# autosome-ru/pasio

Measured on NVIDIA B200. Metric: whole-contig segmentation throughput, default pasio pipeline (nt/s); DP cell updates/s in dp_cells_per_s, higher is better.
Workload: dtype f64

## Files before the change

pasio_b200/csrc/window_dp.cu:

```cuda
#include "dp_core.cuh"
#include "bound.cuh"
#include <cstdio>
#include <cstdlib>

namespace {

constexpr int WD_THREADS = 256;
constexpr int WD_WARPS = WD_THREADS / 32;
constexpr int WD_FARW = WD_WARPS - 1;
constexpr int NEAR_Q = 4;
constexpr int PR_CB = 32;
constexpr int PR_FB = 8;
constexpr int PR_MIN_N = 256;
constexpr int PR_DENSE = 28;

#ifdef PASIO_WD_PROF
__device__ unsigned long long g_wd_prof[16];
struct ProfAcc { long long t0; long long a0, a1, a2, a3, a4, a5, a6, a7; };
#define PROF_DECL ProfAcc prof = {clock64(), 0, 0, 0, 0, 0, 0, 0, 0}
__device__ __forceinline__ long long prof_clock()
{
    unsigned dummy;
    long long t;
    asm volatile("ld.volatile.shared.u32 %0, [%1];" : "=r"(dummy) : "r"(0u) : "memory");
    asm volatile("mov.u64 %0, %%clock64;" : "=l"(t) : "r"(dummy) : "memory");
    return t;
}
#define PROF_T(i) do { const long long t1__ = prof_clock(); prof.a##i += t1__ - prof.t0; prof.t0 = t1__; } while (0)
#define PROF_FLUSH do { if (threadIdx.x == 0 || threadIdx.x == 32) { unsigned long long *g__ = g_wd_prof + (threadIdx.x ? 8 : 0); \
    atomicAdd(g__ + 0, (unsigned long long)prof.a0); atomicAdd(g__ + 1, (unsigned long long)prof.a1); \
    atomicAdd(g__ + 2, (unsigned long long)prof.a2); atomicAdd(g__ + 3, (unsigned long long)prof.a3); \
    atomicAdd(g__ + 4, (unsigned long long)prof.a4); atomicAdd(g__ + 5, (unsigned long long)prof.a5); \
    atomicAdd(g__ + 6, (unsigned long long)prof.a6); atomicAdd(g__ + 7, (unsigned long long)prof.a7); } \
    prof.a0 = prof.a1 = prof.a2 = prof.a3 = prof.a4 = prof.a5 = prof.a6 = prof.a7 = 0; } while (0)
#define PROF_ARGS , ProfAcc &prof
#define PROF_PASS , prof
#else
#define PROF_DECL
#define PROF_T(i) do { } while (0)
#define PROF_FLUSH do { } while (0)
#define PROF_ARGS
#define PROF_PASS
#endif

struct WinDpParams {
    WinGeom geom;
    i64 nwin;
    const int32_t *cand;
    const i64 *cg;
    const i64 *cgc;
    const uint32_t *cpbits;
    uint32_t *keepbits;
    const double *gtab;
    const double *ltab;
    int constraint;
    int alpha_int;
    double alpha;
    double pen;
    int cap;
    u64 *cells;
    u64 *cells_skipped;
    unsigned *work_counter;
    const int32_t *list;
    i64 w_begin;
    i64 n_p1, list_len;
    unsigned char *done_flags;
    int p1_stride;
    int skip_covered;
    int speculate;
    int n_lg;
};

__host__ __device__ inline size_t window_smem_bytes(int cap)
{
    const size_t capr = (size_t)((cap + 31) & ~31);
    return capr * 16
           + NEAR_Q * 32 * 8
           + DP_JB * DP_JB * 8
           + NEAR_Q * 32 * 4
           + 24 * 4
           + capr * 2
           + (capr / PR_CB) * sizeof(CoarseRec)
           + 2 * 32 * sizeof(float4)
           + capr * 2
           + 2 * ((capr / PR_CB) * 2 + 16)
           + 2 * WD_FARW * 32 * (8 + 4)
           + 8 * 8;
}

__device__ __forceinline__ int2 col_lc(const ColRec *sCol, int i)
{
    return *reinterpret_cast<const int2 *>(sCol + i);
}

template <bool AI>
__device__ __forceinline__ void compute_row_lb(int jbp, int jb, int N, const ColRec *sCol, float4 *sRow, double *sRowStat,
                                               double delta_path, double pen,
                                               const double *__restrict__ gtab, const double *__restrict__ ltab,
                                               int alpha_int, double alpha)
{
    const int lane = threadIdx.x & 31;
    const int jrow = min(jb + lane, N - 1);
    const int2 me = col_lc(sCol, jrow);
    const RowConst<AI> rme = make_row<AI>(me.y, me.x, alpha_int, alpha);
    const int jp = jbp + lane;
    const int2 pm = col_lc(sCol, jp), pb = col_lc(sCol, jp - 1), before = col_lc(sCol, jrow - 1);
    const RowConst<AI> rp = make_row<AI>(pm.y, pm.x, alpha_int, alpha);
    const double wp = self_score<AI>(pb.y, pb.x, rp, gtab, ltab) + pen;
    double run = self_score<AI>(before.y, before.x, rme, gtab, ltab) + (lane ? pen : 0.0);
    const double tot_prev = warp_sum(wp);
#pragma unroll
    for (int d = 1; d < 32; d <<= 1) {
        const double o = __shfl_up_sync(0xffffffffu, run, d);
        if (lane >= d) run += o;
    }
    double path = (sCol[jbp - 1].P + tot_prev) + run - delta_path;
    if (!(fabs(path) < 1e30)) path = -INFINITY;
    float lbf = (float)path;
    sRow[lane] = make_float4(lbf, (float)me.y, (float)me.x, 0.f);
    double ab = (jb + lane < N && path > -1e300) ? fabs(path) : 0.0;
#pragma unroll
    for (int off = 16; off > 0; off >>= 1) ab = fmax(ab, __shfl_xor_sync(0xffffffffu, ab, off));
    if (lane == 0) *sRowStat = ab;
}

__device__ __forceinline__ double tilted_row_min(const float4 *sRow, int r0, int r1, double a, double b, double lbabs,
                                                 int c_max, int l_max)
{
    const float af = (float)a, bf = (float)b;
    float m = INFINITY;
#pragma unroll 4
    for (int r = r0; r <= r1; ++r) {
        const float4 rr = sRow[r];
        m = fminf(m, fmaf(af, rr.y, fmaf(bf, rr.z, rr.x)));
    }
    const double err = (lbabs + fabs(a) * (double)c_max + fabs(b) * (double)l_max) * 9.5367431640625e-07;
    return (double)m - err;
}

template <bool AI>
__device__ __forceinline__ u64 far_pass(int jb, int N, int nfar, const ColRec *sCol, const CoarseRec *sCoarse,
                                        const float4 *sRow, double lbabs, unsigned short *sList, unsigned short *sDense,
                                        unsigned short *sSurv, int *sListCount ,
                                        double *sFarVW, int *sFarAW, double delta,
                                        const double *__restrict__ gtab, const double *__restrict__ ltab,
                                        int alpha_int, double alpha PROF_ARGS)
{
    const int lane = threadIdx.x & 31, w7 = (threadIdx.x >> 5) - 1;
    const int nrows = min(DP_JB, N - jb);
    const int2 rowF = col_lc(sCol, jb), rowL = col_lc(sCol, jb + nrows - 1);
    const int2 me = col_lc(sCol, min(jb + lane, N - 1));
    const RowConst<AI> rme = make_row<AI>(me.y, me.x, alpha_int, alpha);

    double best = -INFINITY;
    int arg = 0x7fffffff;
    if (w7 == 0 && lane < nrows) {
        const ColRec a0 = sCol[0];
        best = __dadd_rn(self_score<AI>(a0.C, a0.L, rme, gtab, ltab), a0.P);
        arg = 0;
    }
    u64 skipped = 0;

    const int rg = lane >> 2, q = lane & 3;
    const int r0 = 4 * rg, r1 = min(r0 + 3, nrows - 1);
    const bool act2 = r0 < nrows;
    const int2 gF = col_lc(sCol, jb + min(r0, nrows - 1)), gL = col_lc(sCol, jb + r1);

    auto level2 = [&](int cb1) {
        const CoarseRec *rec = sCoarse + cb1;
        const double a = rec->a, b = rec->b;
        bool surv2 = false;
        if (act2) {
            const int i0 = 1 + PR_CB * cb1 + PR_FB * q;
            const int2 cF = col_lc(sCol, i0), cL = col_lc(sCol, i0 + PR_FB - 1);
            const double m2 = tilted_box_max<AI>(gF.y - cL.y, gL.y - cF.y, gF.x - cL.x, gL.x - cF.x, a, b,
                                                 gtab, ltab, alpha_int, alpha);
            const double m3 = tilted_row_min(sRow, r0, r1, a, b, lbabs, gL.y, gL.x);
            surv2 = !(rec->mpt8[q] + m2 - m3 + delta < 0.0);
            if (!surv2) skipped += (u64)(PR_FB * (r1 - r0 + 1));
        }
        const unsigned mask2 = __ballot_sync(0xffffffffu, surv2);
        const int n2 = __popc(mask2);
        if (n2 >= PR_DENSE) {
            if (act2 && !surv2) skipped -= (u64)(PR_FB * (r1 - r0 + 1));
            if (lane == 0) sDense[atomicAdd(sListCount + 1, 1)] = (unsigned short)cb1;
        } else if (n2) {
            int slot = 0;
            if (lane == 0) slot = atomicAdd(sListCount, n2);
            slot = __shfl_sync(0xffffffffu, slot, 0);
            if (surv2) sList[slot + __popc(mask2 & ((1u << lane) - 1u))] = (unsigned short)((cb1 << 5) | lane);
        }
    };
    const int l1_warps = min(WD_FARW, (nfar + 31) / 32);
    const int n_direct = max(0, min(nfar, WD_FARW - l1_warps));
    const int nfar1 = nfar - n_direct;
    if (w7 >= l1_warps && w7 - l1_warps < n_direct) level2(nfar - 1 - (w7 - l1_warps));

    for (int base = 0; base + 32 * w7 < nfar1 && w7 < l1_warps; base += 32 * l1_warps) {
        const int cb = base + 32 * w7 + lane;
        bool surv1 = false;
        if (cb < nfar1) {
            const CoarseRec *rec = sCoarse + cb;
            const int4 ends = *reinterpret_cast<const int4 *>(rec);
            const double a1 = rec->a, b1 = rec->b;
            const double ub1 = rec->mpt + tilted_box_max<AI>(rowF.y - ends.y, rowL.y - ends.x, rowF.x - ends.w, rowL.x - ends.z,
                                                             a1, b1, gtab, ltab, alpha_int, alpha);
            const double m3 = tilted_row_min(sRow, 0, nrows - 1, a1, b1, lbabs, rowL.y, rowL.x);
            surv1 = !(ub1 - m3 + delta < 0.0);
            if (!surv1) skipped += (u64)(PR_CB * nrows);
        }
        const unsigned mask1 = __ballot_sync(0xffffffffu, surv1);
        if (mask1) {
            int slot = 0;
            if (lane == 0) slot = atomicAdd(sListCount + 2, __popc(mask1));
            slot = __shfl_sync(0xffffffffu, slot, 0);
            if (surv1) sSurv[slot + __popc(mask1 & ((1u << lane) - 1u))] = (unsigned short)cb;
        }
    }
    PROF_T(4);
    asm volatile("bar.sync 1, %0;" ::"n"(WD_FARW * 32) : "memory");
    const int nsurv = *reinterpret_cast<volatile int *>(sListCount + 2);

    for (int e = w7; e < nsurv; e += WD_FARW) level2(sSurv[e]);
    PROF_T(5);
    asm volatile("bar.sync 1, %0;" ::"n"(WD_FARW * 32) : "memory");
    const int total = *reinterpret_cast<volatile int *>(sListCount);
    const int ndense = *reinterpret_cast<volatile int *>(sListCount + 1);
    PROF_T(3);

    for (int e = w7; e < ndense; e += WD_FARW) {
        const int i0 = 1 + PR_CB * (int)sDense[e];
        const int rr = lane & 3, cph = lane >> 2;
#pragma unroll 1
        for (int g = 0; g < 4; ++g) {
            RowConst<AI> r[2];
            double bst[2];
            int ag[2];
#pragma unroll
            for (int k = 0; k < 2; ++k) {
                const int2 rl = col_lc(sCol, min(jb + g * 8 + k * 4 + rr, N - 1));
                r[k] = make_row<AI>(rl.y, rl.x, alpha_int, alpha);
                bst[k] = -INFINITY;
                ag[k] = i0 + cph;
            }
            sweep_columns<AI, 4, 2>(i0, i0 + PR_CB, cph, 8, sCol, r, gtab, ltab, bst, ag);
#pragma unroll
            for (int k = 0; k < 2; ++k) {
                merge_column_phases<4>(bst[k], ag[k]);
                const double v = __shfl_sync(0xffffffffu, bst[k], lane & 3);
                const int va = __shfl_sync(0xffffffffu, ag[k], lane & 3);
                if ((lane >> 2) == g * 2 + k && lane < nrows && (v > best || (v == best && va < arg))) { best = v; arg = va; }
            }
        }
    }

    constexpr int UX = 4;
    const int er = lane >> 3, ec = lane & 7;
    for (int e0 = w7 * UX; e0 < total; e0 += WD_FARW * UX) {
        double t[UX];
        int ta[UX], g4[UX];
#pragma unroll
        for (int u = 0; u < UX; ++u) {
            t[u] = -INFINITY;
            ta[u] = 0x7fffffff;
            g4[u] = 0;
            if (e0 + u < total) {
                const int ent = sList[e0 + u];
                const int l2 = ent & 31;
                g4[u] = 4 * (l2 >> 2);
                const int row = g4[u] + er;
                const int col = 1 + PR_CB * (ent >> 5) + PR_FB * (l2 & 3) + ec;
                ta[u] = col;
                if (row < nrows) {
                    const int2 rl = col_lc(sCol, jb + row);
                    const RowConst<AI> rc = make_row<AI>(rl.y, rl.x, alpha_int, alpha);
                    const ColRec cc = sCol[col];
                    t[u] = __dadd_rn(self_score<AI>(cc.C, cc.L, rc, gtab, ltab), cc.P);
                }
            }
        }
#pragma unroll
        for (int u = 0; u < UX; ++u) {
#pragma unroll
            for (int off = 1; off < 8; off <<= 1) {
                const double ob = __shfl_xor_sync(0xffffffffu, t[u], off);
                const int oa = __shfl_xor_sync(0xffffffffu, ta[u], off);
                if (ob > t[u] || (ob == t[u] && oa < ta[u])) { t[u] = ob; ta[u] = oa; }
            }
            const int rel = lane - g4[u];
            const double v = __shfl_sync(0xffffffffu, t[u], (rel & 3) * 8);
            const int va = __shfl_sync(0xffffffffu, ta[u], (rel & 3) * 8);
            if (rel >= 0 && rel < 4 && (v > best || (v == best && va < arg))) { best = v; arg = va; }
        }
    }
    sFarVW[lane] = best;
    sFarAW[lane] = arg;
    return skipped;
}

template <bool AI, int NW>
__device__ __forceinline__ void near_tri_farwarps(int w7 , int jb, int N, const ColRec *sCol, double *sPartV,
                                                  int *sPartA, double *sTri,
                                                  const double *__restrict__ gtab, const double *__restrict__ ltab,
                                                  int alpha_int, double alpha)
{
    const int lane = threadIdx.x & 31;
    const int rr = lane & 3, cc = lane >> 2;
    constexpr int NT = (16 + NW - 1) / NW;
    double tv[NT][2];
    int tcol[NT];
#pragma unroll
    for (int u = 0; u < NT; ++u) {
        const int t = w7 + u * NW;
        const int grp = t & 3, qc = (t >> 2) & 3;
        tcol[u] = jb - PR_CB + qc * 8 + cc;
        const ColRec a = sCol[tcol[u]];
#pragma unroll
        for (int k = 0; k < 2; ++k) {
            const int j = min(jb + grp * 8 + k * 4 + rr, N - 1);
            const int2 me = col_lc(sCol, j);
            const RowConst<AI> r = make_row<AI>(me.y, me.x, alpha_int, alpha);
            tv[u][k] = (t < 16) ? __dadd_rn(self_score<AI>(a.C, a.L, r, gtab, ltab), a.P) : -INFINITY;
        }
    }
    const int2 mt = col_lc(sCol, min(jb + lane, N - 1));
    const RowConst<AI> rt = make_row<AI>(mt.y, mt.x, alpha_int, alpha);
    constexpr int NK = (DP_JB + NW - 1) / NW;
    double w[NK];
#pragma unroll
    for (int kk = 0; kk < NK; ++kk) {
        const int k = w7 + kk * NW;
        w[kk] = 0.0;
        if (k < lane && jb + lane < N) {
            const int2 a = col_lc(sCol, jb + k);
            w[kk] = self_score<AI>(a.y, a.x, rt, gtab, ltab);
        }
    }
#pragma unroll
    for (int u = 0; u < NT; ++u) {
        const int t = w7 + u * NW;
#pragma unroll
        for (int k = 0; k < 2; ++k) {
            double best = tv[u][k];
            int arg = tcol[u];
            merge_column_phases<4>(best, arg);
            if (cc == 0 && t < 16) {
                const int row = (t & 3) * 8 + k * 4 + rr;
                sPartV[(t >> 2) * 32 + row] = best;
                sPartA[(t >> 2) * 32 + row] = arg;
            }
        }
    }
#pragma unroll
    for (int kk = 0; kk < NK; ++kk) {
        const int k = w7 + kk * NW;
        if (k < lane && jb + lane < N) sTri[k * DP_JB + lane] = w[kk];
    }
}

__device__ __forceinline__ void build_coarse_record(int jb, const ColRec *sCol, CoarseRec *rec, double tilt_scale_c,
                                                    double tilt_scale_l)
{
    const ColRec me = sCol[jb + (threadIdx.x & 31)];
    fit_column_record(me.C, me.L, me.P, rec, tilt_scale_c, tilt_scale_l);
}

template <bool AI, int U, int RPL, bool PRUNE>
__global__ void __launch_bounds__(WD_THREADS, 3)
window_dp_kernel(WinDpParams p)
{
    extern __shared__ __align__(16) unsigned char smem[];
    const int capr = (p.cap + 31) & ~31;
    ColRec *sCol = reinterpret_cast<ColRec *>(smem);
    double *sPartV = reinterpret_cast<double *>(sCol + capr);
    double *sTri = sPartV + NEAR_Q * 32;
    int *sPartA = reinterpret_cast<int *>(sTri + DP_JB * DP_JB);
    int *sMisc = sPartA + NEAR_Q * 32;
    unsigned short *sPrev = reinterpret_cast<unsigned short *>(sMisc + 24);
    CoarseRec *sCoarse = reinterpret_cast<CoarseRec *>(sPrev + capr);
    float4 *sRow = reinterpret_cast<float4 *>(sCoarse + capr / PR_CB);
    double *sFarV = reinterpret_cast<double *>(sRow + 2 * 32);
    int *sFarA = reinterpret_cast<int *>(sFarV + 2 * WD_FARW * 32);
    double *sScal = reinterpret_cast<double *>(sFarA + 2 * WD_FARW * 32);
    unsigned short *sList = reinterpret_cast<unsigned short *>(sScal + 8);
    int *sListCount = sMisc + 16;
    unsigned short *sJump = reinterpret_cast<unsigned short *>(sCoarse);
    unsigned char *sMark = reinterpret_cast<unsigned char *>(sTri);

    const int tid = threadIdx.x, lane = tid & 31, warp = tid >> 5;
    PROF_DECL;

    while (true) {
        PROF_T(7);
        PROF_FLUSH;
        if (tid == 0) sMisc[0] = (int)atomicAdd(p.work_counter, 1u);
        __syncthreads();
        const i64 widx = (unsigned)sMisc[0];
        if (widx >= p.nwin) break;
        const bool second = widx >= p.n_p1;
        const bool phase2 = second && p.skip_covered;
        const i64 w = !p.list ? p.w_begin + widx
                              : (second ? (i64)__ldg(p.list + (p.list_len - 1 - (widx - p.n_p1))) : (i64)__ldg(p.list + widx));
        if (phase2) {
            if (tid == 0) {
                const i64 rel = w - p.w_begin, lo = rel - rel % p.p1_stride, hi = lo + p.p1_stride;
                const volatile unsigned char *f = p.done_flags;
                while (!f[lo] || (hi < p.list_len && !f[hi])) __nanosleep(200);
                __threadfence();
                i64 skip_cells = -1;
                if (hi < p.list_len && (f[lo] & 2) && (f[hi] & 2)) {
                    i64 s0, e0, s1, e1, s2, e2;
                    window_range(p.geom, w, s0, e0);
                    window_range(p.geom, p.w_begin + lo, s1, e1);
                    window_range(p.geom, p.w_begin + hi, s2, e2);
                    if (s1 <= s0 && e1 >= s2 && e2 >= e0) skip_cells = (e0 - s0) * (e0 - s0 - 1) / 2;
                }
                if (skip_cells >= 0) {
                    atomicAdd(p.cells, (u64)skip_cells);
                    atomicAdd(p.cells_skipped, (u64)skip_cells);
                }
                sMisc[1] = skip_cells >= 0;
            }
            __syncthreads();
            if (sMisc[1]) continue;
        }
        int kept_all = 1;

        i64 st, en;
        window_range(p.geom, w, st, en);
        const int nq = (int)(en - st);
        const i64 first = p.cand ? (i64)__ldg(p.cand + st) : st;
        const i64 last = p.cand ? (i64)__ldg(p.cand + en - 1) : en - 1;
        const i64 cg_first = p.cand ? __ldg(p.cgc + st) : __ldg(p.cg + first);
        const bool all_zero = (p.constraint == PASIO_CONSTRAINT_ZEROS) && ((p.cand ? __ldg(p.cgc + en - 1) : __ldg(p.cg + last)) == cg_first);
        int count = 0;
        const bool by_words = !p.cand && p.constraint == PASIO_CONSTRAINT_CONSTANTS;
        if (by_words) {
            const i64 w0 = first >> 5, w1 = last >> 5;
            const int nwords = (int)(w1 - w0 + 1);
            for (int base = 0; base < nwords; base += WD_THREADS) {
                const int t = base + tid;
                unsigned word = 0;
                if (t < nwords) {
                    word = __ldg(p.cpbits + w0 + t);
                    if (t == 0) word = (word & (0xffffffffu << (first & 31))) | (1u << (first & 31));
                    if (t == nwords - 1) word = (word & (0xffffffffu >> (31 - (last & 31)))) | (1u << (last & 31));
                }
                int incl = __popc(word);
                const int mine = incl;
#pragma unroll
                for (int d = 1; d < 32; d <<= 1) {
                    const int o = __shfl_up_sync(0xffffffffu, incl, d);
                    if (lane >= d) incl += o;
                }
                if (lane == 31) sMisc[4 + warp] = incl;
                __syncthreads();
                int woff = 0, tot = 0;
#pragma unroll
                for (int w2 = 0; w2 < WD_WARPS; ++w2) {
                    const int c = sMisc[4 + w2];
                    if (w2 < warp) woff += c;
                    tot += c;
                }
                int k = count + woff + incl - mine;
                const i64 pos0 = (w0 + t) << 5;
                while (word) {
                    const i64 pos = pos0 + (__ffs(word) - 1);
                    word &= word - 1;
                    sCol[k].L = (int)(pos - first);
                    sCol[k].C = (int)(__ldg(p.cg + pos) - cg_first);
                    ++k;
                }
                count += tot;
                __syncthreads();
            }
        }
        for (int base = 0; !by_words && base < nq; base += WD_THREADS) {
            const int q = base + tid;
            i64 pos = 0;
            bool take = false;
            if (q < nq) {
                pos = p.cand ? (i64)__ldg(p.cand + st + q) : st + q;
                if (q == 0 || q == nq - 1 || p.constraint == PASIO_CONSTRAINT_NONE) take = true;
                else if (p.constraint == PASIO_CONSTRAINT_CONSTANTS) take = bit_test(p.cpbits, pos);
                else take = !all_zero;
                if (phase2 && !((__ldcg(p.keepbits + (pos >> 5)) >> (pos & 31)) & 1u)) kept_all = 0;
            }
            const unsigned bal = __ballot_sync(0xffffffffu, take);
            if (lane == 0) sMisc[4 + warp] = __popc(bal);
            __syncthreads();
            int woff = 0, tot = 0;
#pragma unroll
            for (int w2 = 0; w2 < WD_WARPS; ++w2) {
                const int c = sMisc[4 + w2];
                if (w2 < warp) woff += c;
                tot += c;
            }
            if (take) {
                const int k = count + woff + __popc(bal & ((1u << lane) - 1u));
                sCol[k].L = (int)(pos - first);
                sCol[k].C = (int)((p.cand ? __ldg(p.cgc + st + q) : __ldg(p.cg + pos)) - cg_first);
            }
            count += tot;
            __syncthreads();
        }
        const int N = count;
        PROF_T(0);
        if (phase2 && __syncthreads_and(kept_all)) {
            if (tid == 0) {
                const u64 c = (u64)N * (u64)(N - 1) / 2;
                atomicAdd(p.cells, c);
                atomicAdd(p.cells_skipped, c);
            }
            continue;
        }

        if (tid == 0) { sCol[0].P = 0.0; sPrev[0] = 0; }
        __syncthreads();
        u64 skipped = 0;
        if (PRUNE && tid == 0) {
            const ColRec z = sCol[N - 1];
            const int x = z.C + (AI ? p.alpha_int : 0);
            sScal[0] = fabs(__ldg(p.gtab + x)) + ((double)z.C + p.alpha) * fabs(__ldg(p.ltab + z.L)) + 1.0;
            sScal[1] = 0.0;
            sScal[2] = (double)z.C + p.alpha;
            sScal[3] = (double)z.L;
        }
        auto finish_block = [&](int jb) {
            if (jb + DP_JB <= N) build_coarse_record(jb, sCol, sCoarse + (jb - 1) / PR_CB, sScal[2], sScal[3]);
            double ab = jb + lane < N ? fabs(sCol[jb + lane].P) : 0.0;
#pragma unroll
            for (int off = 16; off > 0; off >>= 1) ab = fmax(ab, __shfl_xor_sync(0xffffffffu, ab, off));
            if (lane == 0) sScal[1] = fmax(sScal[1], ab);
        };
        auto far_delta = [&]() { return (sScal[0] + sScal[1] + fabs(p.pen) * DP_JB) * 5.684341886080802e-14; };
        auto prepare_rows = [&](int jbn) {
            const int par = ((jbn - 1) / DP_JB) & 1;
            const double delta_path = (sScal[0] + sScal[1] + fabs(p.pen) * DP_JB) * 1.8189894035458565e-12;
            compute_row_lb<AI>(jbn - DP_JB, jbn, N, sCol, sRow + 32 * par, sScal + 4 + par, delta_path, p.pen, p.gtab, p.ltab,
                               p.alpha_int, p.alpha);
            if (lane == 0) { sListCount[4 * par] = 0; sListCount[4 * par + 1] = 0; sListCount[4 * par + 2] = 0; }
        };
        auto run_far = [&](int jbf) {
            const int kf = (jbf - 1) / DP_JB, par = kf & 1;
            skipped += far_pass<AI>(jbf, N, kf - 1, sCol, sCoarse, sRow + 32 * par, sScal[4 + par], sList, sList + capr,
                                    sList + capr + capr / PR_CB + 8, sListCount + 4 * par, sFarV + (par * WD_FARW + warp - 1) * 32,
                                    sFarA + (par * WD_FARW + warp - 1) * 32,
                                    far_delta(), p.gtab, p.ltab, p.alpha_int, p.alpha PROF_PASS);
        };
        int jb = 1;
        const bool pipelined = PRUNE && N > PR_MIN_N && p.cand != nullptr;
        for (; jb < N && (!pipelined || jb < 1 + 2 * DP_JB); jb += DP_JB) {
            dp_block_step<AI, WD_WARPS, U, RPL>(jb, N, 0, sCol, sPrev, nullptr, sPartV, sPartA, sTri,
                                                p.gtab, p.ltab, p.alpha_int, p.alpha, p.pen, -INFINITY, 0, 0);
            if (pipelined && warp == 0) finish_block(jb);
        }
        PROF_T(6);
        if (pipelined && jb < N) {
            int spec_wait = 0, spec_back = 1;
            if (warp == 0) prepare_rows(jb);
            __syncthreads();
            if (warp > 0) run_far(jb);
            else if (jb + DP_JB < N) prepare_rows(jb + DP_JB);
            __syncthreads();
            for (; jb < N; jb += DP_JB) {
                const int k = (jb - 1) / DP_JB, buf = k & 1;
                near_tri_farwarps<AI, WD_WARPS>(warp, jb, N, sCol, sPartV, sPartA, sTri, p.gtab, p.ltab, p.alpha_int, p.alpha);
                PROF_T(1);
                __syncthreads();
                PROF_T(6);
                if (warp == 0) {
                    double fbest = -INFINITY;
                    int farg = 0;
#pragma unroll
                    for (int w2 = 0; w2 < WD_FARW; ++w2) {
                        const double v = sFarV[(buf * WD_FARW + w2) * 32 + lane];
                        const int a = sFarA[(buf * WD_FARW + w2) * 32 + lane];
                        if (v > fbest || (v == fbest && a < farg)) { fbest = v; farg = a; }
                    }
                    const double ib = jb + lane < N ? fbest : -INFINITY;
                    const int ia = jb + lane < N ? farg : 0;
                    bool resolved = false;
                    if (p.speculate && spec_wait == 0) {
                        resolved = block_chain_speculative<NEAR_Q>(jb, N, sCol, sPrev, sPartV, sPartA, sTri, p.pen, ib, ia);
                        if (resolved) spec_back = 1;
                        else { spec_wait = spec_back; spec_back = min(spec_back * 2, 16); }
                    } else if (spec_wait > 0) {
                        --spec_wait;
                    }
                    if (!resolved) block_chain<NEAR_Q>(jb, N, sCol, sPrev, nullptr, sPartV, sPartA, sTri, p.pen, ib, ia, 0, nullptr);
                    __syncwarp();
                    finish_block(jb);
                    if (jb + 2 * DP_JB < N) prepare_rows(jb + 2 * DP_JB);
                } else if (jb + DP_JB < N) {
                    run_far(jb + DP_JB);
                }
                PROF_T(2);
                __syncthreads();
                PROF_T(7);
            }
        }

        for (int k = tid; k < N; k += WD_THREADS) sMark[k] = (k == N - 1);
        __syncthreads();
        unsigned short *ja = sPrev, *jb2 = sJump;
        for (int reach = 1; reach < N; reach <<= 1) {
            for (int k = tid; k < N; k += WD_THREADS)
                if (sMark[k]) sMark[ja[k]] = 1;
            for (int k = tid; k < N; k += WD_THREADS) jb2[k] = ja[ja[k]];
            __syncthreads();
            unsigned short *t = ja; ja = jb2; jb2 = t;
        }
        int every = N == nq;
        for (int k = tid; k < N; k += WD_THREADS) {
            if (sMark[k]) {
                const i64 pos = first + sCol[k].L;
                atomicOr(p.keepbits + (pos >> 5), 1u << (pos & 31));
            } else {
                every = 0;
            }
        }
        if (!second && p.skip_covered && p.n_p1 < p.nwin) {
            __threadfence();
            every = __syncthreads_and(every);
            if (tid == 0) {
                __threadfence();
                *reinterpret_cast<volatile unsigned char *>(p.done_flags + (w - p.w_begin)) = every ? 3 : 1;
            }
        }
        if (tid == 0) atomicAdd(p.cells, (u64)N * (u64)(N - 1) / 2);
        if (PRUNE) {
#pragma unroll
            for (int off = 16; off > 0; off >>= 1) skipped += __shfl_xor_sync(0xffffffffu, skipped, off);
            if (lane == 0 && skipped) atomicAdd(p.cells_skipped, skipped);
        }
        __syncthreads();
    }
}

constexpr int SW_JB = 16;
constexpr int SW_SMALL_N = WD_SMALL_MAX_CANDIDATES, SW_SMALL_WARPS = 8, SW_SMALL_CTAS = 5;
constexpr int SW_MEDIUM_N = WD_MEDIUM_MAX_CANDIDATES, SW_MEDIUM_WARPS = 4, SW_MEDIUM_CTAS = 4;

template <int MAXN>
struct __align__(16) SmallWin {
    ColRec col[MAXN];
    double tri[SW_JB * SW_JB];
    unsigned short prev[MAXN];
    unsigned char mark[MAXN];
};

template <bool AI, int MAXN, int NWARPS, int CTAS, int U, bool LGS>
__global__ void __launch_bounds__(NWARPS * 32, CTAS)
small_window_dp_kernel(WinDpParams p)
{
    extern __shared__ __align__(16) unsigned char smem[];
    const int lane = threadIdx.x & 31;
    SmallWin<MAXN> &W = reinterpret_cast<SmallWin<MAXN> *>(smem)[threadIdx.x >> 5];
    u64 my_cells = 0;
    const double *lgt = p.ltab;
    if (LGS) {
        double *sLg = reinterpret_cast<double *>(smem + sizeof(SmallWin<MAXN>) * NWARPS);
        for (int k = threadIdx.x; k < p.n_lg; k += NWARPS * 32) sLg[k] = __ldg(p.ltab + k);
        __syncthreads();
        lgt = sLg;
    }

    while (true) {
        unsigned widx = 0;
        if (lane == 0) widx = atomicAdd(p.work_counter, 1u);
        widx = __shfl_sync(0xffffffffu, widx, 0);
        if ((i64)widx >= p.nwin) break;
        const i64 w = __ldg(p.list + widx);

        i64 st, en;
        window_range(p.geom, w, st, en);
        const int nq = (int)(en - st);
        const i64 first = p.cand ? (i64)__ldg(p.cand + st) : st;
        const i64 last = p.cand ? (i64)__ldg(p.cand + en - 1) : en - 1;
        const i64 cg_first = p.cand ? __ldg(p.cgc + st) : __ldg(p.cg + first);
        const bool all_zero = (p.constraint == PASIO_CONSTRAINT_ZEROS) && ((p.cand ? __ldg(p.cgc + en - 1) : __ldg(p.cg + last)) == cg_first);
        int count = 0;
        if (!p.cand && p.constraint == PASIO_CONSTRAINT_CONSTANTS) {
            const i64 w0 = first >> 5, w1 = last >> 5;
            const int nwords = (int)(w1 - w0 + 1);
            for (int base = 0; base < nwords; base += 32) {
                const int t = base + lane;
                unsigned word = 0;
                if (t < nwords) {
                    word = __ldg(p.cpbits + w0 + t);
                    if (t == 0) word = (word & (0xffffffffu << (first & 31))) | (1u << (first & 31));
                    if (t == nwords - 1) word = (word & (0xffffffffu >> (31 - (last & 31)))) | (1u << (last & 31));
                }
                int incl = __popc(word);
                const int mine = incl;
#pragma unroll
                for (int d = 1; d < 32; d <<= 1) {
                    const int o = __shfl_up_sync(0xffffffffu, incl, d);
                    if (lane >= d) incl += o;
                }
                int k = count + incl - mine;
                const i64 pos0 = (w0 + t) << 5;
                while (word) {
                    const i64 pos = pos0 + (__ffs(word) - 1);
                    word &= word - 1;
                    W.col[k].L = (int)(pos - first);
                    W.col[k].C = (int)(__ldg(p.cg + pos) - cg_first);
                    ++k;
                }
                count += __shfl_sync(0xffffffffu, incl, 31);
            }
        } else {
            for (int base = 0; base < nq; base += 32) {
                const int q = base + lane;
                i64 pos = 0;
                bool take = false;
                if (q < nq) {
                    pos = p.cand ? (i64)__ldg(p.cand + st + q) : st + q;
                    if (q == 0 || q == nq - 1 || p.constraint == PASIO_CONSTRAINT_NONE) take = true;
                    else if (p.constraint == PASIO_CONSTRAINT_CONSTANTS) take = bit_test(p.cpbits, pos);
                    else take = !all_zero;
                }
                const unsigned bal = __ballot_sync(0xffffffffu, take);
                if (take) {
                    const int k = count + __popc(bal & ((1u << lane) - 1u));
                    W.col[k].L = (int)(pos - first);
                    W.col[k].C = (int)((p.cand ? __ldg(p.cgc + st + q) : __ldg(p.cg + pos)) - cg_first);
                }
                count += __popc(bal);
            }
        }
        const int N = count;
        if (lane == 0) { W.col[0].P = 0.0; W.prev[0] = 0; }
        __syncwarp();

        const int r = lane & 15, ph = lane >> 4;
        for (int jb = 1; jb < N; jb += SW_JB) {
            const ColRec me = W.col[min(jb + r, N - 1)];
            RowConst<AI> rc[1] = {make_row<AI>(me.C, me.L, p.alpha_int, p.alpha)};
            double best[1] = {-INFINITY};
            int arg[1] = {ph};
            sweep_columns<AI, U, 1, LGS>(0, jb, ph, 2, W.col, rc, p.gtab, lgt, best, arg);
            {
                const double ob = __shfl_xor_sync(0xffffffffu, best[0], 16);
                const int oa = __shfl_xor_sync(0xffffffffu, arg[0], 16);
                if (ob > best[0] || (ob == best[0] && oa < arg[0])) { best[0] = ob; arg[0] = oa; }
            }
            for (int k = ph; k < r; k += 2)
                if (jb + r < N) {
                    const ColRec a = W.col[jb + k];
                    W.tri[k * SW_JB + r] = self_score<AI, LGS>(a.C, a.L, rc[0], p.gtab, lgt);
                }
            __syncwarp();
            double bst = best[0], mine = 0.0;
            int ag = arg[0];
            const int rows = min(SW_JB, N - jb);
#pragma unroll 4
            for (int k = 0; k < rows; ++k) {
                const double pf = __dadd_rn(bst, p.pen);
                const double pk = __shfl_sync(0xffffffffu, pf, k);
                if (r == k) mine = pf;
                if (r > k) {
                    const double t = __dadd_rn(W.tri[k * SW_JB + r], pk);
                    if (t > bst) { bst = t; ag = jb + k; }
                }
            }
            if (lane < SW_JB && jb + r < N) {
                W.col[jb + r].P = mine;
                W.prev[jb + r] = (unsigned short)ag;
            }
            __syncwarp();
        }

        for (int k = lane; k < N; k += 32) W.mark[k] = 0;
        __syncwarp();
        if (lane == 0) {
            int k = N - 1;
            while (true) {
                W.mark[k] = 1;
                if (k == 0) break;
                k = W.prev[k];
            }
        }
        __syncwarp();
        for (int k = lane; k < N; k += 32)
            if (W.mark[k]) {
                const i64 pos = first + W.col[k].L;
                atomicOr(p.keepbits + (pos >> 5), 1u << (pos & 31));
            }
        my_cells += (u64)N * (u64)(N - 1) / 2;
        __syncwarp();
    }
    if (lane == 0 && my_cells) atomicAdd(p.cells, my_cells);
}

}

int small_window_max_candidates() { return SW_SMALL_N; }
int medium_window_max_candidates() { return SW_MEDIUM_N; }

int window_dp_max_candidates(pasio_ctx *ctx)
{
    int cap = 32;
    while (cap + 32 <= 8192 && window_smem_bytes(cap + 32) <= (size_t)ctx->smem_optin) cap += 32;
    return cap;
}

int launch_window_dp(pasio_ctx *ctx, i64 nwin, int wsize, int wshift, int constraint, i64 w_begin, bool keep_cell_counters)
{
    WinDpParams p;
    p.geom = make_geom(ctx, wsize, wshift);
    p.nwin = nwin;
    p.cand = cur_cand(ctx);
    p.cg = ctx->cg.as<i64>();
    p.cgc = cur_cand_cg(ctx);
    p.cpbits = ctx->cpbits.as<uint32_t>();
    p.keepbits = ctx->keepbits.as<uint32_t>();
    p.gtab = ctx->tab[ctx->alpha_is_int ? PASIO_TAB_LGAMMA : PASIO_TAB_LGAMMA_ALPHA].as<double>();
    p.ltab = ctx->tab[PASIO_TAB_LOG].as<double>();
    p.constraint = constraint;
    p.alpha_int = (int)ctx->alpha_int;
    p.alpha = ctx->alpha;
    p.pen = ctx->pen;
    i64 cap = (i64)wsize + 1;
    if (cap > ctx->m) cap = ctx->m;
    if (cap > 8192 || window_smem_bytes((int)cap) > (size_t)ctx->smem_optin)
        return pasio_fail(ctx, PASIO_E_TOO_LARGE, "window of %lld candidates does not fit one CTA's shared memory (max %d)",
                          (long long)cap, window_dp_max_candidates(ctx));
    p.cap = (int)cap;
    p.cells = ctx->scalars.as<u64>() + 10;
    p.cells_skipped = ctx->scalars.as<u64>() + 12;
    p.work_counter = ctx->scalars.as<unsigned>() + 2 * 11;
    p.w_begin = w_begin;
    if (keep_cell_counters) CUDA_TRY(ctx, cudaMemsetAsync(ctx->scalars.as<u64>() + 11, 0, 8, ctx->stream));
    else CUDA_TRY(ctx, cudaMemsetAsync(ctx->scalars.as<u64>() + 10, 0, 24, ctx->stream));
    CUDA_TRY(ctx, cudaMemsetAsync(ctx->scalars.as<u64>() + 15, 0, 8, ctx->stream));

    static const int small_env = getenv("PASIO_WD_SMALL") ? atoi(getenv("PASIO_WD_SMALL")) : 1;
    const int phase_env = ctx->tune[PASIO_TUNE_WINDOW_PHASES];
    const bool use_lists = small_env && ctx->n_small + ctx->n_medium + ctx->n_large == nwin;
    const i64 n_small = use_lists ? ctx->n_small : 0, n_medium = use_lists ? ctx->n_medium : 0;
    const i64 n_large = use_lists ? ctx->n_large : nwin;
    p.list = use_lists ? ctx->win_large.as<int32_t>() : nullptr;
    p.nwin = n_large;
    p.list_len = nwin;
    p.n_p1 = use_lists ? ctx->n_large_p1 : n_large;
    p.skip_covered = phase_env;
    p.speculate = ctx->tune[PASIO_TUNE_WINDOW_SPECULATE];
    p.done_flags = ctx->win_flags.as<unsigned char>();
    p.p1_stride = wshift > 0 && wsize / wshift > 1 ? wsize / wshift : 1;
    if (!use_lists) p.skip_covered = 0;
    ctx->n_small = ctx->n_medium = ctx->n_large = ctx->n_large_p1 = -1;
    TimingScope ts_all(ctx, TF_WINDOW_DP, 0);
    const bool fork = n_small + n_medium > 0 && n_small + n_medium <= 64;
    const bool serial_small = n_small + n_medium > 64;
    if (fork) CUDA_TRY(ctx, cudaEventRecord(ctx->ev_fork, ctx->stream));

    auto launch_small = [&](auto kern, const int32_t *list, i64 n, int nwarps, int ctas, size_t smem_bytes, unsigned *counter,
                            cudaStream_t stream) -> int {
        if (n <= 0) return PASIO_OK;
        WinDpParams ps = p;
        ps.list = list;
        ps.nwin = n;
        ps.n_p1 = n;
        ps.work_counter = counter;
        CUDA_TRY(ctx, cudaFuncSetAttribute(kern, cudaFuncAttributeMaxDynamicSharedMemorySize, (int)smem_bytes));
        int resident = ctas;
        CUDA_TRY(ctx, cudaOccupancyMaxActiveBlocksPerMultiprocessor(&resident, kern, nwarps * 32, smem_bytes));
        if (resident < 1) resident = 1;
        if (resident > ctas) resident = ctas;
        i64 g = (n + nwarps - 1) / nwarps;
        if (g > (i64)ctx->sm_count * resident) g = (i64)ctx->sm_count * resident;
        ctx->fam_launches[TF_WINDOW_DP] += 1;
        kern<<<(unsigned)g, nwarps * 32, smem_bytes, stream>>>(ps);
        CUDA_TRY(ctx, cudaGetLastError());
        return PASIO_OK;
    };
    static const int lgs_env = getenv("PASIO_WD_LGS") ? atoi(getenv("PASIO_WD_LGS")) : 0;
    const bool lgs = lgs_env && p.cand == nullptr && (i64)wsize + 2 <= 4096 && ctx->ntab[PASIO_TAB_LOG] >= (i64)wsize + 2;
    p.n_lg = lgs ? wsize + 2 : 0;
    const size_t lg_bytes = (size_t)((p.n_lg + 1) & ~1) * 8;
    auto launch_small_kernels = [&](cudaStream_t stream) -> int {
        unsigned *c_small = ctx->scalars.as<unsigned>() + 2 * 15, *c_medium = c_small + 1;
        const size_t sm_small = sizeof(SmallWin<SW_SMALL_N>) * SW_SMALL_WARPS + lg_bytes,
                     sm_medium = sizeof(SmallWin<SW_MEDIUM_N>) * SW_MEDIUM_WARPS + lg_bytes;
#define PASIO_SMALL_LAUNCH(AIV, LGV)                                                                                                          \
        PASIO_TRY(launch_small(small_window_dp_kernel<AIV, SW_SMALL_N, SW_SMALL_WARPS, SW_SMALL_CTAS, 4, LGV>, ctx->win_small.as<int32_t>(),   \
                               n_small, SW_SMALL_WARPS, SW_SMALL_CTAS, sm_small, c_small, stream));                                            \
        PASIO_TRY(launch_small(small_window_dp_kernel<AIV, SW_MEDIUM_N, SW_MEDIUM_WARPS, SW_MEDIUM_CTAS, 8, LGV>, ctx->win_medium.as<int32_t>(), \
                               n_medium, SW_MEDIUM_WARPS, SW_MEDIUM_CTAS, sm_medium, c_medium, stream));
        if (ctx->alpha_is_int) {
            if (lgs) { PASIO_SMALL_LAUNCH(true, true) } else { PASIO_SMALL_LAUNCH(true, false) }
        } else {
            if (lgs) { PASIO_SMALL_LAUNCH(false, true) } else { PASIO_SMALL_LAUNCH(false, false) }
        }
#undef PASIO_SMALL_LAUNCH
        return PASIO_OK;
    };
    if (serial_small) PASIO_TRY(launch_small_kernels(ctx->stream));

    i64 grid = 0;
    if (n_large > 0) {
        const size_t smem = window_smem_bytes(p.cap);
        const int prune_env = ctx->tune[PASIO_TUNE_WINDOW_PRUNE];
        const bool prune = prune_env != 0 && ctx->alpha >= 0.0009765625;
        void (*kern)(WinDpParams);
        if (ctx->alpha_is_int) kern = prune ? window_dp_kernel<true, 4, 2, true> : window_dp_kernel<true, 4, 2, false>;
        else kern = prune ? window_dp_kernel<false, 4, 2, true> : window_dp_kernel<false, 4, 2, false>;
        CUDA_TRY(ctx, cudaFuncSetAttribute(kern, cudaFuncAttributeMaxDynamicSharedMemorySize, (int)smem));
        int per_sm = 0;
        CUDA_TRY(ctx, cudaOccupancyMaxActiveBlocksPerMultiprocessor(&per_sm, kern, WD_THREADS, smem));
        if (per_sm < 1) per_sm = 1;
#ifdef PASIO_WD_PROF
        if (getenv("PASIO_WD_CTAS") && atoi(getenv("PASIO_WD_CTAS")) < per_sm) per_sm = atoi(getenv("PASIO_WD_CTAS"));
#endif
        grid = (i64)ctx->sm_count * per_sm;
        if (grid > n_large) grid = n_large;
        if (grid < 1) grid = 1;
        ctx->fam_launches[TF_WINDOW_DP] += 1;
        kern<<<(unsigned)grid, WD_THREADS, smem, ctx->stream>>>(p);
        CUDA_TRY(ctx, cudaGetLastError());
    }
    if (fork) {
        CUDA_TRY(ctx, cudaStreamWaitEvent(ctx->stream2, ctx->ev_fork, 0));
        PASIO_TRY(launch_small_kernels(ctx->stream2));
        CUDA_TRY(ctx, cudaEventRecord(ctx->ev_join, ctx->stream2));
        CUDA_TRY(ctx, cudaStreamWaitEvent(ctx->stream, ctx->ev_join, 0));
    }
#ifdef PASIO_WD_PROF
    {
        cudaStreamSynchronize(ctx->stream);
        unsigned long long h[16], z[16] = {0};
        cudaMemcpyFromSymbol(h, g_wd_prof, sizeof h);
        cudaMemcpyToSymbol(g_wd_prof, z, sizeof z);
        static const char *names[8] = {"compact", "X:work", "Y:work(chain|far L3)", "far:listwait", "far:L1", "far:L2", "wait@X+plain", "wait@Y+rest"};
        for (int side = 0; side < 2; ++side) {
            double tot = 0;
            for (int i = 0; i < 8; ++i) tot += (double)h[8 * side + i];
            fprintf(stderr, "[wd_prof %s] nwin=%lld grid=%lld:", side ? "warp1" : "warp0", (long long)nwin, (long long)grid);
            for (int i = 0; i < 8; ++i) if (h[8 * side + i]) fprintf(stderr, " %s=%.1f%%", names[i], 100.0 * (double)h[8 * side + i] / tot);
            fprintf(stderr, " | cycles/CTA=%.3g\n", tot / (double)grid);
        }
    }
#endif
    return PASIO_OK;
}
```

Baseline: 5.702 billion.

## Prefetch next block's row-bound and first far-box table loads during near phase

Splits the row lower-bound computation and the first level-1 tilted box bound into a load phase and a compute phase. The global table loads (gtab/ltab) for the next block's row scores (warp 0) and for each far warp's first coarse box are issued before near_tri_farwarps, so their latency overlaps the near-triangle work. The results are consumed after the barrier. This adds register pressure and some duplicated index computation in exchange for hiding global-load latency on the critical pipelined path.

```diff
diff --git a/pasio_b200/csrc/window_dp.cu b/pasio_b200/csrc/window_dp.cu
--- a/pasio_b200/csrc/window_dp.cu
+++ b/pasio_b200/csrc/window_dp.cu
@@ -93,11 +93,25 @@
     return *reinterpret_cast<const int2 *>(sCol + i);
 }
 
+struct ScoreLoads { double g, lg, s; };
 template <bool AI>
-__device__ __forceinline__ void compute_row_lb(int jbp, int jb, int N, const ColRec *sCol, float4 *sRow, double *sRowStat,
-                                               double delta_path, double pen,
-                                               const double *__restrict__ gtab, const double *__restrict__ ltab,
-                                               int alpha_int, double alpha)
+__device__ __forceinline__ ScoreLoads self_score_loads(int ci, int li, const RowConst<AI> &r,
+                                                       const double *__restrict__ gtab, const double *__restrict__ ltab)
+{
+    const int idx = r.cjx - ci;
+    ScoreLoads l;
+    l.g = __ldg(gtab + idx);
+    l.lg = __ldg(ltab + (r.lj - li));
+    l.s = AI ? u32_to_double(idx) : __dsub_rn(r.aj, u32_to_double(ci));
+    return l;
+}
+__device__ __forceinline__ double self_score_of(const ScoreLoads &l) { return __dsub_rn(l.g, __dmul_rn(l.s, l.lg)); }
+
+struct RowLbLoads { ScoreLoads prev, run; };
+template <bool AI>
+__device__ __forceinline__ RowLbLoads row_lb_loads(int jbp, int jb, int N, const ColRec *sCol,
+                                                   const double *__restrict__ gtab, const double *__restrict__ ltab,
+                                                   int alpha_int, double alpha)
 {
     const int lane = threadIdx.x & 31;
     const int jrow = min(jb + lane, N - 1);
@@ -106,8 +120,26 @@
     const int jp = jbp + lane;
     const int2 pm = col_lc(sCol, jp), pb = col_lc(sCol, jp - 1), before = col_lc(sCol, jrow - 1);
     const RowConst<AI> rp = make_row<AI>(pm.y, pm.x, alpha_int, alpha);
-    const double wp = self_score<AI>(pb.y, pb.x, rp, gtab, ltab) + pen;
-    double run = self_score<AI>(before.y, before.x, rme, gtab, ltab) + (lane ? pen : 0.0);
+    RowLbLoads l;
+    l.prev = self_score_loads<AI>(pb.y, pb.x, rp, gtab, ltab);
+    l.run = self_score_loads<AI>(before.y, before.x, rme, gtab, ltab);
+    return l;
+}
+
+struct RowLbScores { double prev, run; };
+__device__ __forceinline__ RowLbScores row_lb_scores(const RowLbLoads &ld)
+{
+    return RowLbScores{self_score_of(ld.prev), self_score_of(ld.run)};
+}
+
+__device__ __forceinline__ void compute_row_lb(int jbp, int jb, int N, const ColRec *sCol, float4 *sRow, double *sRowStat,
+                                               double delta_path, double pen, const RowLbScores &w)
+{
+    const int lane = threadIdx.x & 31;
+    const int jrow = min(jb + lane, N - 1);
+    const int2 me = col_lc(sCol, jrow);
+    const double wp = w.prev + pen;
+    double run = w.run + (lane ? pen : 0.0);
     const double tot_prev = warp_sum(wp);
 #pragma unroll
     for (int d = 1; d < 32; d <<= 1) {
@@ -122,6 +154,45 @@
 #pragma unroll
     for (int off = 16; off > 0; off >>= 1) ab = fmax(ab, __shfl_xor_sync(0xffffffffu, ab, off));
     if (lane == 0) *sRowStat = ab;
+}
+
+__device__ __forceinline__ void level1_split(int nfar, int &l1_warps, int &n_direct, int &nfar1)
+{
+    l1_warps = min(WD_FARW, (nfar + 31) / 32);
+    n_direct = max(0, min(nfar, WD_FARW - l1_warps));
+    nfar1 = nfar - n_direct;
+}
+
+__device__ __forceinline__ int4 level1_box(int jb, int N, int cb, const ColRec *sCol, const CoarseRec *sCoarse)
+{
+    const int nrows = min(DP_JB, N - jb);
+    const int2 rowF = col_lc(sCol, jb), rowL = col_lc(sCol, jb + nrows - 1);
+    const int4 ends = *reinterpret_cast<const int4 *>(sCoarse + cb);
+    return make_int4(rowF.y - ends.y, rowL.y - ends.x, rowF.x - ends.w, rowL.x - ends.z);
+}
+
+__device__ __forceinline__ int level1_first_block(int jb)
+{
+    int l1_warps, n_direct, nfar1;
+    level1_split((jb - 1) / DP_JB - 1, l1_warps, n_direct, nfar1);
+    const int cb = 32 * ((threadIdx.x >> 5) - 1) + (threadIdx.x & 31);
+    return max(0, min(cb, nfar1 - 1));
+}
+template <bool AI>
+__device__ __forceinline__ BoxCorners level1_first_loads(int jb, int N, const ColRec *sCol, const CoarseRec *sCoarse,
+                                                         const double *__restrict__ gtab, const double *__restrict__ ltab,
+                                                         int alpha_int)
+{
+    const int4 bx = level1_box(jb, N, level1_first_block(jb), sCol, sCoarse);
+    return box_corner_loads<AI>(bx.x, bx.y, bx.z, bx.w, gtab, ltab, alpha_int);
+}
+__device__ __forceinline__ double level1_first_box(int jb, int N, const ColRec *sCol, const CoarseRec *sCoarse,
+                                                   const BoxCorners &c, double alpha)
+{
+    const int cb = level1_first_block(jb);
+    const int4 bx = level1_box(jb, N, cb, sCol, sCoarse);
+    const CoarseRec *rec = sCoarse + cb;
+    return rec->mpt + tilted_box_max_of(c, bx.x, bx.y, bx.z, bx.w, rec->a, rec->b, alpha);
 }
 
 __device__ __forceinline__ double tilted_row_min(const float4 *sRow, int r0, int r1, double a, double b, double lbabs,
@@ -144,7 +215,7 @@
                                         unsigned short *sSurv, int *sListCount ,
                                         double *sFarVW, int *sFarAW, double delta,
                                         const double *__restrict__ gtab, const double *__restrict__ ltab,
-                                        int alpha_int, double alpha PROF_ARGS)
+                                        int alpha_int, double alpha, const double *first_box PROF_ARGS)
 {
     const int lane = threadIdx.x & 31, w7 = (threadIdx.x >> 5) - 1;
     const int nrows = min(DP_JB, N - jb);
@@ -191,9 +262,8 @@
             if (surv2) sList[slot + __popc(mask2 & ((1u << lane) - 1u))] = (unsigned short)((cb1 << 5) | lane);
         }
     };
-    const int l1_warps = min(WD_FARW, (nfar + 31) / 32);
-    const int n_direct = max(0, min(nfar, WD_FARW - l1_warps));
-    const int nfar1 = nfar - n_direct;
+    int l1_warps, n_direct, nfar1;
+    level1_split(nfar, l1_warps, n_direct, nfar1);
     if (w7 >= l1_warps && w7 - l1_warps < n_direct) level2(nfar - 1 - (w7 - l1_warps));
 
     for (int base = 0; base + 32 * w7 < nfar1 && w7 < l1_warps; base += 32 * l1_warps) {
@@ -203,8 +273,10 @@
             const CoarseRec *rec = sCoarse + cb;
             const int4 ends = *reinterpret_cast<const int4 *>(rec);
             const double a1 = rec->a, b1 = rec->b;
-            const double ub1 = rec->mpt + tilted_box_max<AI>(rowF.y - ends.y, rowL.y - ends.x, rowF.x - ends.w, rowL.x - ends.z,
-                                                             a1, b1, gtab, ltab, alpha_int, alpha);
+            const double ub1 = (first_box && base == 0)
+                                   ? *first_box
+                                   : rec->mpt + tilted_box_max<AI>(rowF.y - ends.y, rowL.y - ends.x, rowF.x - ends.w,
+                                                                   rowL.x - ends.z, a1, b1, gtab, ltab, alpha_int, alpha);
             const double m3 = tilted_row_min(sRow, 0, nrows - 1, a1, b1, lbabs, rowL.y, rowL.x);
             surv1 = !(ub1 - m3 + delta < 0.0);
             if (!surv1) skipped += (u64)(PR_CB * nrows);
@@ -534,19 +606,20 @@
             if (lane == 0) sScal[1] = fmax(sScal[1], ab);
         };
         auto far_delta = [&]() { return (sScal[0] + sScal[1] + fabs(p.pen) * DP_JB) * 5.684341886080802e-14; };
-        auto prepare_rows = [&](int jbn) {
+        auto prepare_rows = [&](int jbn, const RowLbScores &w) {
             const int par = ((jbn - 1) / DP_JB) & 1;
             const double delta_path = (sScal[0] + sScal[1] + fabs(p.pen) * DP_JB) * 1.8189894035458565e-12;
-            compute_row_lb<AI>(jbn - DP_JB, jbn, N, sCol, sRow + 32 * par, sScal + 4 + par, delta_path, p.pen, p.gtab, p.ltab,
-                               p.alpha_int, p.alpha);
+            compute_row_lb(jbn - DP_JB, jbn, N, sCol, sRow + 32 * par, sScal + 4 + par, delta_path, p.pen, w);
             if (lane == 0) { sListCount[4 * par] = 0; sListCount[4 * par + 1] = 0; sListCount[4 * par + 2] = 0; }
         };
-        auto run_far = [&](int jbf) {
+        auto row_loads = [&](int jbn) { return row_lb_loads<AI>(jbn - DP_JB, jbn, N, sCol, p.gtab, p.ltab, p.alpha_int, p.alpha); };
+        auto row_scores = [&](int jbn) { return row_lb_scores(row_loads(jbn)); };
+        auto run_far = [&](int jbf, const double *first_box) {
             const int kf = (jbf - 1) / DP_JB, par = kf & 1;
             skipped += far_pass<AI>(jbf, N, kf - 1, sCol, sCoarse, sRow + 32 * par, sScal[4 + par], sList, sList + capr,
                                     sList + capr + capr / PR_CB + 8, sListCount + 4 * par, sFarV + (par * WD_FARW + warp - 1) * 32,
                                     sFarA + (par * WD_FARW + warp - 1) * 32,
-                                    far_delta(), p.gtab, p.ltab, p.alpha_int, p.alpha PROF_PASS);
+                                    far_delta(), p.gtab, p.ltab, p.alpha_int, p.alpha, first_box PROF_PASS);
         };
         int jb = 1;
         const bool pipelined = PRUNE && N > PR_MIN_N && p.cand != nullptr;
@@ -558,14 +631,23 @@
         PROF_T(6);
         if (pipelined && jb < N) {
             int spec_wait = 0, spec_back = 1;
-            if (warp == 0) prepare_rows(jb);
+            if (warp == 0) prepare_rows(jb, row_scores(jb));
             __syncthreads();
-            if (warp > 0) run_far(jb);
-            else if (jb + DP_JB < N) prepare_rows(jb + DP_JB);
+            if (warp > 0) run_far(jb, nullptr);
+            else if (jb + DP_JB < N) prepare_rows(jb + DP_JB, row_scores(jb + DP_JB));
             __syncthreads();
             for (; jb < N; jb += DP_JB) {
                 const int k = (jb - 1) / DP_JB, buf = k & 1;
+                RowLbLoads rl = {};
+                BoxCorners bc = {};
+                if (warp == 0) {
+                    if (jb + 2 * DP_JB < N) rl = row_loads(jb + 2 * DP_JB);
+                } else if (jb + DP_JB < N) {
+                    bc = level1_first_loads<AI>(jb + DP_JB, N, sCol, sCoarse, p.gtab, p.ltab, p.alpha_int);
+                }
                 near_tri_farwarps<AI, WD_WARPS>(warp, jb, N, sCol, sPartV, sPartA, sTri, p.gtab, p.ltab, p.alpha_int, p.alpha);
+                const double first_box = warp > 0 && jb + DP_JB < N ? level1_first_box(jb + DP_JB, N, sCol, sCoarse, bc, p.alpha) : 0.0;
+                const RowLbScores rw = row_lb_scores(rl);
                 PROF_T(1);
                 __syncthreads();
                 PROF_T(6);
@@ -591,9 +673,9 @@
                     if (!resolved) block_chain<NEAR_Q>(jb, N, sCol, sPrev, nullptr, sPartV, sPartA, sTri, p.pen, ib, ia, 0, nullptr);
                     __syncwarp();
                     finish_block(jb);
-                    if (jb + 2 * DP_JB < N) prepare_rows(jb + 2 * DP_JB);
+                    if (jb + 2 * DP_JB < N) prepare_rows(jb + 2 * DP_JB, rw);
                 } else if (jb + DP_JB < N) {
-                    run_far(jb + DP_JB);
+                    run_far(jb + DP_JB, &first_box);
                 }
                 PROF_T(2);
                 __syncthreads();
```

New measurement: 5.208 billion (median of 6 runs). -8.7%, worse.
